# B3zaleel/draco-sharp

Measured on AMD Instinct MI355X. Metric: decoded_meshes_per_sec, higher is better.
Workload: dtype int32

## Files before the change

### draco-sharp_amd/csrc/dsa_kernels.h

```cpp
#pragma once
#include <hip/hip_runtime.h>
#include <stdint.h>

#include "dsa_common.h"
#include "dsa_locate.h"
#include "dsa_needs.h"
#ifdef DSA_EXPERIMENTS
#include "dsa_lanes.h"
#else
#define LN_FLAG_SYMBOLS 1u
#define LN_FLAG_PREDICT 2u
#define LN_FLAG_OCT 8u
namespace dsa { namespace lanes {
__device__ __forceinline__ bool ln_sym_eligible(const AttrDesc &, const MeshLayout &, uint32_t, uint32_t) { return false; }
__device__ __forceinline__ bool ln_oct_eligible(const AttrDesc &, uint32_t) { return false; }
} }
#endif

#ifndef DSA_CHAIN_PRIO
#define DSA_CHAIN_PRIO 3
#endif

namespace dsa {

__device__ __forceinline__ uint32_t cnext(uint32_t c) { return (c % 3u == 2u) ? c - 2u : c + 1u; }
__device__ __forceinline__ uint32_t cprev(uint32_t c) { return (c % 3u == 0u) ? c + 2u : c - 1u; }
__device__ __forceinline__ uint32_t uni(uint32_t v) { return (uint32_t)__builtin_amdgcn_readfirstlane((int)v); }
__device__ __forceinline__ uint32_t lane_id() { return threadIdx.x & 63u; }
template <class T>
__device__ __forceinline__ T *uni_ptr(T *p) {
  const uint64_t v = (uint64_t)p;
  return (T *)(((uint64_t)(uint32_t)__builtin_amdgcn_readfirstlane((int)(uint32_t)(v >> 32)) << 32) | (uint32_t)__builtin_amdgcn_readfirstlane((int)(uint32_t)v));
}
__device__ __forceinline__ uint32_t rdlane(uint32_t v, uint32_t l) { return (uint32_t)__builtin_amdgcn_readlane((int)v, (int)l); }
#define LATE_HANDOFF 0x40000u
__device__ __forceinline__ void late_handoff(uint8_t *arena, const MeshLayout &L, MeshDesc *D, uint32_t ai, uint32_t flags, uint32_t bit);
__device__ __forceinline__ uint64_t clk() { return __builtin_amdgcn_s_memtime(); }
__device__ __forceinline__ uint64_t realclk() { return __builtin_amdgcn_s_memrealtime(); }
__device__ __forceinline__ uint32_t leading_lanes(bool pred) { uint64_t m = ~__ballot(pred); return m ? (uint32_t)__builtin_ctzll(m) : 64u; }
#define WAIT_VM0() __builtin_amdgcn_s_waitcnt(0x0F70)

template <int CTRL>
__device__ __forceinline__ uint32_t dpp_mov(uint32_t x) { return (uint32_t)__builtin_amdgcn_update_dpp(0, (int)x, CTRL, 0xF, 0xF, false); }
__device__ __forceinline__ uint32_t lane_prev(uint32_t x) { return dpp_mov<0x138>(x); }
template <class Op>
__device__ __forceinline__ uint32_t wave_incl_scan(uint32_t x, Op op) {
  const uint32_t lane = lane_id(), rl = lane & 15u;
  uint32_t t;
  t = dpp_mov<0x111>(x); if (rl >= 1) x = op(t, x);
  t = dpp_mov<0x112>(x); if (rl >= 2) x = op(t, x);
  t = dpp_mov<0x114>(x); if (rl >= 4) x = op(t, x);
  t = dpp_mov<0x118>(x); if (rl >= 8) x = op(t, x);
  t = dpp_mov<0x142>(x); if ((lane & 31u) >= 16) x = op(t, x);
  t = dpp_mov<0x143>(x); if (lane >= 32) x = op(t, x);
  return x;
}
__device__ __forceinline__ uint32_t wave_excl_scan(uint32_t v, uint32_t *total) {
  const uint32_t x = wave_incl_scan(v, [](uint32_t a, uint32_t b) { return a + b; });
  *total = rdlane(x, 63);
  return x - v;
}

template <bool CP> struct Rec;
struct FaceIds { uint32_t v0, v1, v2, o0, o1, o2; };
template <> struct Rec<false> {
  static constexpr uint32_t WORDS = 8;
  struct Raw { uint4 v, o; };
  static __device__ __forceinline__ Raw load(const uint32_t *frec, uint32_t f) { Raw r; r.v = ((const uint4 *)frec)[(size_t)f * 2]; r.o = ((const uint4 *)frec)[(size_t)f * 2 + 1]; return r; }
  static __device__ __forceinline__ Raw none() { Raw r; r.v = make_uint4(0, 0, 0, 0); r.o = make_uint4(DSA_INVALID, DSA_INVALID, DSA_INVALID, 0); return r; }
  static __device__ __forceinline__ Raw or_none(bool ok, const Raw &x) { return ok ? x : none(); }
  static __device__ __forceinline__ uint32_t sel3(uint32_t k, uint32_t x, uint32_t y, uint32_t z) { return k == 0 ? x : (k == 1 ? y : z); }
  static __device__ __forceinline__ uint32_t vertex(const Raw &r, uint32_t k) { return sel3(k, r.v.x, r.v.y, r.v.z); }
  static __device__ __forceinline__ uint32_t opp(const Raw &r, uint32_t k) { return sel3(k, r.o.x, r.o.y, r.o.z); }
  static __device__ __forceinline__ uint32_t get_v(const uint32_t *frec, uint32_t c) { return frec[fv_idx(c)]; }
  static __device__ __forceinline__ uint32_t get_o(const uint32_t *frec, uint32_t c) { return frec[fo_idx(c)]; }
  static __device__ __forceinline__ uint32_t get_o_plain(const uint32_t *frec, uint32_t c) { return frec[fo_idx(c)]; }
  static __device__ __forceinline__ void set_v(uint32_t *frec, uint32_t c, uint32_t val) { frec[fv_idx(c)] = val; }
  static __device__ __forceinline__ void link(uint32_t *frec, uint32_t c, uint32_t val) { frec[fo_idx(c)] = val; }
  static __device__ __forceinline__ void link_lds(uint32_t *stage, uint32_t c_rel, uint32_t val) { stage[fo_idx(c_rel)] = val; }
  static __device__ __forceinline__ void store(uint32_t *frec, uint32_t f, const FaceIds &x) {
    ((uint4 *)frec)[(size_t)f * 2] = make_uint4(x.v0, x.v1, x.v2, 0u); ((uint4 *)frec)[(size_t)f * 2 + 1] = make_uint4(x.o0, x.o1, x.o2, 0u);
  }
  static __device__ __forceinline__ void store_lds(uint32_t *stage, uint32_t slot, const FaceIds &x) {
    *(uint4 *)&stage[slot * 8] = make_uint4(x.v0, x.v1, x.v2, 0u); *(uint4 *)&stage[slot * 8 + 4] = make_uint4(x.o0, x.o1, x.o2, 0u);
  }
  static __device__ __forceinline__ uint4 vertices_of(const uint32_t *frec, uint32_t f) { return ((const uint4 *)frec)[(size_t)f * 2]; }
};
template <> struct Rec<true> {
  static constexpr uint32_t WORDS = 4;
  static constexpr uint32_t M = 0x1FFFFFu;
  struct Raw { uint64_t v, o; };
  static __device__ __forceinline__ uint64_t pack(uint32_t a, uint32_t b, uint32_t c) { return (uint64_t)(a & M) | ((uint64_t)(b & M) << 21) | ((uint64_t)(c & M) << 42); }
  static __device__ __forceinline__ uint32_t field(uint64_t w, uint32_t k) { return (uint32_t)((int32_t)((uint32_t)(w >> (21u * k)) << 11) >> 11); }
  static __device__ __forceinline__ Raw load(const uint32_t *frec, uint32_t f) { const uint4 q = ((const uint4 *)frec)[f]; Raw r; r.v = (uint64_t)q.x | ((uint64_t)q.y << 32); r.o = (uint64_t)q.z | ((uint64_t)q.w << 32); return r; }
  static __device__ __forceinline__ Raw none() { Raw r; r.v = 0; r.o = ~0ull; return r; }
  static __device__ __forceinline__ Raw or_none(bool ok, const Raw &x) { Raw r; r.v = ok ? x.v : 0ull; r.o = ok ? x.o : ~0ull; return r; }
  static __device__ __forceinline__ uint32_t vertex(const Raw &r, uint32_t k) { return field(r.v, k); }
  static __device__ __forceinline__ uint32_t opp(const Raw &r, uint32_t k) { return field(r.o, k); }
  static __device__ __forceinline__ uint32_t get_v(const uint32_t *frec, uint32_t c) { return field(((const uint64_t *)frec)[(size_t)(c >> 2) * 2], c & 3u); }
  static __device__ __forceinline__ uint32_t get_o(const uint32_t *frec, uint32_t c) {
    return field(__hip_atomic_load((const unsigned long long *)frec + (size_t)(c >> 2) * 2 + 1, __ATOMIC_RELAXED, __HIP_MEMORY_SCOPE_AGENT), c & 3u);
  }
  static __device__ __forceinline__ uint32_t get_o_plain(const uint32_t *frec, uint32_t c) { return field(((const uint64_t *)frec)[(size_t)(c >> 2) * 2 + 1], c & 3u); }
  static __device__ __forceinline__ void set_v(uint32_t *frec, uint32_t c, uint32_t val) {
    uint64_t *w = (uint64_t *)frec + (size_t)(c >> 2) * 2;
    const uint32_t sh = 21u * (c & 3u);
    *w = (*w & ~((uint64_t)M << sh)) | ((uint64_t)(val & M) << sh);
  }
  static __device__ __forceinline__ void link(uint32_t *frec, uint32_t c, uint32_t val) {
    const uint32_t sh = 21u * (c & 3u);
    atomicAnd((unsigned long long *)frec + (size_t)(c >> 2) * 2 + 1, ((unsigned long long)(val & M) << sh) | ~((unsigned long long)M << sh));
  }
  static __device__ __forceinline__ void link_lds(uint32_t *stage, uint32_t c_rel, uint32_t val) {
    const uint32_t sh = 21u * (c_rel & 3u);
    atomicAnd((unsigned long long *)stage + (size_t)(c_rel >> 2) * 2 + 1, ((unsigned long long)(val & M) << sh) | ~((unsigned long long)M << sh));
  }
  static __device__ __forceinline__ uint4 quad(const FaceIds &x) { const uint64_t v = pack(x.v0, x.v1, x.v2), o = pack(x.o0, x.o1, x.o2); return make_uint4((uint32_t)v, (uint32_t)(v >> 32), (uint32_t)o, (uint32_t)(o >> 32)); }
  static __device__ __forceinline__ void store(uint32_t *frec, uint32_t f, const FaceIds &x) { ((uint4 *)frec)[f] = quad(x); }
  static __device__ __forceinline__ void store_lds(uint32_t *stage, uint32_t slot, const FaceIds &x) { *(uint4 *)&stage[slot * 4] = quad(x); }
  static __device__ __forceinline__ uint4 vertices_of(const uint32_t *frec, uint32_t f) {
    const uint64_t v = ((const uint64_t *)frec)[(size_t)f * 2];
    return make_uint4(field(v, 0), field(v, 1), field(v, 2), 0u);
  }
};
__device__ __forceinline__ uint32_t k_next(uint32_t k) { return k == 2u ? 0u : k + 1u; }
__device__ __forceinline__ uint32_t k_prev(uint32_t k) { return k == 0u ? 2u : k - 1u; }

__device__ __forceinline__ uint8_t *seam_block(uint8_t *arena, const MeshLayout &L, const SeamLayout &g, uint32_t d) {
  return arena + L.seam + g.data + (uint64_t)d * g.data_stride;
}
__device__ __forceinline__ const uint32_t *att_para(uint8_t *arena, const MeshLayout &L, const MeshDesc *D, const AttrDesc &a) {
  if (a.corner_data == 0) return (const uint32_t *)(arena + L.para);
  const SeamLayout g = seam_layout(L.cap_faces, L.cap_vertices, D->num_att_data, L.rec_compact != 0);
  return (const uint32_t *)(seam_block(arena, L, g, (uint32_t)a.corner_data - 1u) + g.para);
}


template <bool TOGGLE>
__device__ __forceinline__ uint32_t rabs_block_to_words(const Rabs &rb, uint32_t count, uint32_t *words) {
  uint32_t state = rb.state, left = rb.off, first = DSA_INVALID;
  const uint32_t p = rb.p;
  const uintptr_t a0 = (uintptr_t)rb.buf + (left ? left - 1u : 0u);
  const uint32_t *wp = (const uint32_t *)(a0 & ~(uintptr_t)3);
  uint32_t sh = (uint32_t)(a0 & 3u) * 8u;
  uint32_t cur = wp[0], nxt = wp[-1];
  uint32_t word = 0, last = 1;
  for (uint32_t i = 0; i < count; ++i) {
    if (state < 4096u && left > 0u) {
      state = state * 256u + ((cur >> sh) & 255u);
      --left;
      if (sh == 0u) { sh = 24u; cur = nxt; --wp; nxt = wp[-1]; } else sh -= 8u;
    }
    const uint32_t quot = state >> 8, rem = state & 255u, xn = quot * p;
    const bool val = rem < p;
    state = val ? xn + rem : state - xn - p;
    if (val && first == DSA_INVALID) first = i;
    if (TOGGLE) { last ^= val ? 0u : 1u; word |= last << (i & 31u); }
    else word |= (val ? 1u : 0u) << (i & 31u);
    if ((i & 31u) == 31u) { words[i >> 5] = word; word = 0; }
  }
  if (count & 31u) words[count >> 5] = word;
  return first;
}

__global__ __launch_bounds__(WAVE, 4) void k_locate(uint8_t *arena, const MeshLayout *layouts, MeshDesc *descs, uint32_t n, BatchGlobals *G) {
  uint32_t mesh = blockIdx.x;
  if (mesh >= n || threadIdx.x != 0) return;
  MeshDesc *D = &descs[mesh];
  locate_mesh(arena, layouts[mesh], D);
  if (D->status != ST_OK || D->general) return;
  locate_attribute_headers(arena, layouts[mesh], D);
  if (D->status != ST_OK) return;
  locate_attribute_values(arena, layouts[mesh], D, G, nullptr, nullptr, LOC_UNTIL_TAGS);
}
__global__ __launch_bounds__(WAVE, 4) void k_locate_resume(uint8_t *arena, const MeshLayout *layouts, MeshDesc *descs, uint32_t n, BatchGlobals *G) {
  __shared__ uint32_t s_cum[LOC_MAX_TAGS + 1];
  __shared__ __attribute__((aligned(16))) uint32_t s_lut[LOC_LDS_WORDS];
  uint32_t mesh = blockIdx.x;
  if (mesh >= n || threadIdx.x != 0) return;
  MeshDesc *D = &descs[mesh];
  if (D->status != ST_OK || D->general || !D->values_pending) return;
  if (D->values_pending == 2 && !D->seam_tables_done) return;
  locate_attribute_values(arena, layouts[mesh], D, G, s_cum, s_lut, LOC_RESUME);
}

#define CN_REC_BLOCKS 8
#define CN_STAGE 32
#define CN_WIN 64

#define CN_CTX_WORDS (6 * 64)
#define CN_LDS_WORDS (CN_STAGE * 8 + CN_REC_BLOCKS * 64 * 2 + CN_WIN + CN_CTX_WORDS)
#define VAL_LM(x_) ((x_) == DSA_INVALID ? DSA_INVALID : ((x_) & 0x1FFFFFu))
#define VAL_OF(x_) ((x_) >> 21)
__device__ __forceinline__ uint32_t val_pack(uint32_t lm, uint32_t val) { return (lm & 0x1FFFFFu) | ((val < 2047u ? val : 2047u) << 21); }
__device__ __forceinline__ bool valence_decode_list(MeshDesc *D, const uint8_t *stream, uint32_t stream_len, uint32_t off_table, uint32_t nsym, uint32_t P,
                                                    uint32_t off_rans, uint32_t size_rans, uint32_t count, uint32_t *out, uint32_t *sh_tmp) {
  const uint32_t lane = lane_id();
  const uint32_t precision = 1u << P, l_base = precision * 4;
  __syncthreads();
  if (lane == 0) { Rd r(stream, stream_len, off_table); if (!read_prob_table(r, nsym, sh_tmp)) fail(D, ST_INVALID, 400); }
  __syncthreads();
  if (status_of(D) != ST_OK) return false;
  const uint32_t pr = lane < nsym ? sh_tmp[lane] : 0u;
  uint32_t tot;
  const uint32_t ex = wave_excl_scan(pr, &tot);
  if (tot != precision) { if (lane == 0) fail(D, ST_INVALID, 401); return false; }
  const uint32_t cum = lane < nsym ? ex : precision;
// ... 1351 lines not shown
          if (pr) { if (k >= nsym) ok = false; else { lds_cum[k] = pr; symtab[k] = i; ++k; } }
        }
      }
      if (!ok || !r.ok || k != nsym) fail(D, ST_INVALID, 400);
    } else if (!read_prob_table(r, nsym, lds_cum)) fail(D, ST_INVALID, 400);
  }
  WAIT_VM0();
  __syncthreads();
  if (status_of(D) != ST_OK) return;
  uint32_t carry = 0;
  for (uint32_t b0 = 0; b0 < nsym; b0 += WAVE) {
    uint32_t i = b0 + lane;
    uint32_t pr = i < nsym ? lds_cum[i] : 0u;
    uint32_t tot;
    uint32_t ex = wave_excl_scan(pr, &tot);
    if (i < nsym) lds_cum[i] = carry + ex;
    carry += tot;
  }
  if (carry != precision) { if (lane == 0) fail(D, ST_INVALID, 401); return; }
  const uint32_t nblocks = (nsym + WAVE - 1) / WAVE;
  for (uint32_t i = nsym + lane; i < nblocks * WAVE + 1; i += WAVE) lds_cum[i] = precision;
  __syncthreads();
  uint32_t coarse = (lane < nblocks) ? lds_cum[lane * WAVE] : precision;
  uint32_t fine0 = lds_cum[lane];
  const uint8_t *buf = stream + a.off_rans;
  uint32_t x, off;
  {
    uint32_t st = 0, o = 0;
    bool ok = rans_init(buf, a.size_rans, l_base, &st, &o);
    if (!ok) { if (lane == 0) fail(D, ST_INVALID, 402); return; }
    x = uni(st); off = uni(o);
  }
  const uintptr_t base_addr = (uintptr_t)buf;
  const uint32_t mis = (uint32_t)(base_addr & 3u);
  const uint32_t *abuf = (const uint32_t *)(base_addr - mis);
  uint32_t chunk = 0xFFFFFFFFu, W = 0;
  const uint32_t mask = precision - 1;
  uint32_t mine = 0;
  for (uint32_t i = 0; i < num_values; ++i) {
    while (x < l_base && off > 0) {
      --off;
      uint32_t q = off + mis;
      uint32_t ch = q >> 8;
      if (ch != chunk) { chunk = ch; W = abuf[(size_t)ch * 64 + lane]; }
      uint32_t byte = (rdlane(W, (q & 255u) >> 2) >> ((q & 3u) * 8)) & 0xFFu;
      x = (x << 8) | byte;
    }
    uint32_t rem = x & mask;
    uint32_t s, cs, nx;
    if (nblocks == 1) {
      uint32_t j = (uint32_t)__popcll(__ballot(fine0 <= rem)) - 1u;
      cs = rdlane(fine0, j);
      nx = (j < 63) ? rdlane(fine0, j + 1) : precision;
      s = j;
    } else {
      uint32_t b = (uint32_t)__popcll(__ballot(coarse <= rem)) - 1u;
      uint32_t v = lds_cum[b * WAVE + lane];
      uint32_t j = (uint32_t)__popcll(__ballot(v <= rem)) - 1u;
      cs = rdlane(v, j);
      nx = (j < 63) ? rdlane(v, j + 1) : rdlane(coarse, b + 1);
      s = b * WAVE + j;
    }
    x = (nx - cs) * (x >> P) + rem - cs;
    if ((i & 63u) == lane) mine = s;
    if ((i & 63u) == 63u) out[i - 63u + lane] = mine;
  }
  uint32_t tail = num_values & 63u;
  if (tail && lane < tail) out[num_values - tail + lane] = mine;
  if (symtab) {
    WAIT_VM0();
    __syncthreads();
    for (uint32_t i = lane; i < num_values; i += WAVE) out[i] = symtab[out[i]];
  }
}

__device__ __forceinline__ void rans_decode_serial(MeshDesc *D, const uint8_t *stream, uint32_t stream_len, const AttrDesc &a, uint32_t num_values,
                                   uint32_t *out, uint32_t *cum ) {
  if (threadIdx.x != 0) return;
  const uint32_t nsym = a.num_symbols, P = a.precision_bits, precision = 1u << P, l_base = precision * 4;
  Rd r(stream, stream_len, a.off_table);
  if (!read_prob_table(r, nsym, cum)) { fail(D, ST_INVALID, 410); return; }
  uint32_t c = 0;
  for (uint32_t i = 0; i < nsym; ++i) { uint32_t pr = cum[i]; cum[i] = c; c += pr; if (c > precision) break; }
  if (c != precision) { fail(D, ST_INVALID, 411); return; }
  cum[nsym] = precision;
  const uint8_t *buf = stream + a.off_rans;
  uint32_t x, off;
  if (!rans_init(buf, a.size_rans, l_base, &x, &off)) { fail(D, ST_INVALID, 412); return; }
  for (uint32_t i = 0; i < num_values; ++i) {
    while (x < l_base && off > 0) x = (x << 8) | buf[--off];
    uint32_t rem = x & (precision - 1);
    uint32_t lo = 0, hi = nsym;
    while (hi - lo > 1) { uint32_t mid = (lo + hi) >> 1; if (cum[mid] <= rem) lo = mid; else hi = mid; }
    uint32_t cs = cum[lo];
    x = (cum[lo + 1] - cs) * (x >> P) + rem - cs;
    out[i] = lo;
  }
}

typedef uint32_t v32u __attribute__((ext_vector_type(32)));

#define SYM_EARLY_FUSE 0x400u
__device__ __forceinline__ void predict_wave(uint8_t *arena, const MeshLayout &L, MeshDesc *D, uint32_t ai, uint32_t phase, uint32_t flags);
__device__ __forceinline__ void predict_wrap_attribute(uint8_t *arena, const MeshLayout &L, MeshDesc *D, uint32_t ai, uint32_t phase, uint32_t flags);
__device__ __forceinline__ void finalize_attribute(uint8_t *arena, const MeshLayout &L, const MeshDesc *D, uint32_t ai, uint32_t phase, uint32_t flags, uint32_t tid, uint32_t stride);
__device__ __forceinline__ void early_tail(uint8_t *arena, const MeshLayout &L, MeshDesc *D, uint32_t ai, uint32_t flags) {
  if (!(flags & SYM_EARLY_FUSE) || D->general) return;
  const AttrDesc &a = D->att[ai];
  if (att_is_late(a)) return;
  WAIT_VM0();
  __threadfence_block();
  __syncthreads();
  if (status_of(D) != ST_OK) return;
  predict_wrap_attribute(arena, L, D, ai, 0u, flags);
  predict_wave(arena, L, D, ai, 0u, flags);
  WAIT_VM0();
  __threadfence_block();
  __syncthreads();
  if (status_of(D) != ST_OK) return;
  finalize_attribute(arena, L, D, ai, 0u, flags, lane_id(), WAVE);
  if (lane_id() == 0) D->att[ai].early_done = 1;
}

__device__ __forceinline__ void late_handoff(uint8_t *arena, const MeshLayout &L, MeshDesc *D, uint32_t ai, uint32_t flags, uint32_t bit) {
  if (!(flags & LATE_HANDOFF) || D->general) return;
  AttrDesc &a = D->att[ai];
  if (!wrap_fast_ok(a, flags) || !att_is_late(a) || att_behind_tables(a) || a.pred_kind != 1) return;
  __builtin_amdgcn_fence(__ATOMIC_RELEASE, "agent");
  __syncthreads();
  uint32_t old = 0;
  if (lane_id() == 0) old = __hip_atomic_fetch_or(&a.late_ready, bit, __ATOMIC_ACQ_REL, __HIP_MEMORY_SCOPE_AGENT);
  old = uni(old);
  if (!(old & (3u ^ bit))) return;
  __builtin_amdgcn_fence(__ATOMIC_ACQUIRE, "agent");
  if (status_of(D) != ST_OK) return;
  predict_wrap_attribute(arena, L, D, ai, 1u, flags);
  WAIT_VM0();
  __syncthreads();
  if (lane_id() == 0) a.late_ready = 7u;
}

#define REG_ATTR 0
#define REG_TAGS 1
#define REG_VLIST 2
#define REG_SCRATCH_BYTES (4096u * 6u + REG_MAX_SYMS * 4u)
#ifdef DSA_SYM_STAMPS
#define REG_STAMP_BEGIN() uint64_t st_t = clk()
#define REG_STAMP(p) { const uint64_t t_ = clk(); if (ATTR && ai < 3 && lane_id() == 0) { const uint32_t k_ = 3u * (p) + ai; \
    ((uint16_t *)D->dbg)[k_ < 6 ? 20 + k_ : 30 + k_] = (uint16_t)((t_ - st_t) >> 10 > 65535 ? 65535 : (t_ - st_t) >> 10); } st_t = t_; }
#else
#define REG_STAMP_BEGIN()
#define REG_STAMP(p)
#endif
__device__ __forceinline__ uint32_t reg_final_symbol(uint32_t v, bool positive) {
  return positive ? v : ((v & 1u) ? (uint32_t)(-(int32_t)(v >> 1) - 1) : (v >> 1));
}
template <int MODE>
__device__ __forceinline__ void reg_decode_stream(uint8_t *arena, const MeshLayout &L, MeshDesc *D, uint32_t ai, uint32_t flags) {
  constexpr bool TAGS = MODE == REG_TAGS, VLIST = MODE == REG_VLIST, ATTR = MODE == REG_ATTR;
  AttrDesc &a = D->att[VLIST ? 0u : ai];
  uint8_t *scratch;
  REG_STAMP_BEGIN();
  uint32_t st_off_table = a.off_table, st_off_rans = a.off_rans, st_size_rans = a.size_rans, st_nsym = a.num_symbols;
  uint32_t st_values = a.num_entries * (TAGS ? 1u : (uint32_t)a.nc_portable);
  uint32_t *out = (uint32_t *)(arena + L.work[VLIST ? 0u : ai]);
  if (VLIST) {
    st_values = D->val_count[ai];
    if (st_values == 0 || D->val_prec[ai] != 12 || D->val_nsym[ai] > 64) return;
    if ((uint64_t)L.rec_compact * 16ull * D->num_faces < 6ull * REG_SCRATCH_BYTES) return;
    st_off_table = D->val_off_table[ai]; st_off_rans = D->val_off_rans[ai]; st_size_rans = D->val_size_rans[ai]; st_nsym = D->val_nsym[ai];
    uint32_t before = 0;
    for (uint32_t k = 0; k < ai; ++k) before += D->val_count[k];
    if ((uint64_t)before + st_values > 3ull * D->num_faces) return;
    out = (uint32_t *)(arena + L.faces) + before;
    scratch = arena + L.frec + (size_t)ai * REG_SCRATCH_BYTES;
  } else if (TAGS) {
    if (a.source != SRC_TAGGED || a.tags_done || a.num_symbols > LOC_MAX_TAGS || a.num_distinct <= 1 || a.num_entries == 0) return;
    const uint64_t slots = ((uint64_t)a.num_entries * 4 + 15) & ~15ull;
    if ((uint64_t)L.work_cap[ai] * 4 < slots + REG_SCRATCH_BYTES) return;
    scratch = arena + L.work[ai] + slots;
  } else {
    if (lanes::ln_sym_eligible(a, L, ai, flags)) return;
    if (sym_filtered(a, flags)) return;
    if (!sym_reg_eligible(a, L, ai)) return;
    scratch = arena + L.out[ai];
  }
  const uint8_t *stream = arena + L.stream;
  uint32_t *slot_tab = (uint32_t *)scratch;
  uint16_t *slot_sym = (uint16_t *)(scratch + 4096 * 4);
  uint32_t *lds = (uint32_t *)(scratch + 4096 * 6);
  const uint32_t lane = lane_id();
  const uint32_t nsym = uni(st_nsym);
  const uint32_t num_values = uni(st_values);
  if (num_values == 0) return;
  if (lane == 0) {
    Rd r(stream, L.stream_len, st_off_table);
    if (!read_prob_table(r, nsym, lds)) fail(D, ST_INVALID, 400);
  }
  __syncthreads();
  if (status_of(D) != ST_OK) return;
  uint32_t carry = 0, one_at = DSA_INVALID;
  bool over = false;
  for (uint32_t b0 = 0; b0 < REG_MAX_SYMS; b0 += WAVE) {
    uint32_t i = b0 + lane;
    uint32_t pr = i < nsym ? lds[i] : 0u;
    if (pr > 4095) { over = true; one_at = i; }
    uint32_t tot;
    uint32_t ex = wave_excl_scan(pr, &tot);
    lds[i] = (pr << 12) | ((carry + ex) & 4095u);
    carry += tot;
    if (carry > 4096) over = true;
  }
  if (VLIST && carry == 4096 && __ballot(over)) {
    uint32_t st = 0, o = 0;
    if (!rans_init(stream + st_off_rans, st_size_rans, 16384, &st, &o)) { if (lane == 0) fail(D, ST_INVALID, 402); return; }
    const uint32_t one = (uint32_t)__builtin_ctzll(__ballot(one_at != DSA_INVALID));
    const uint32_t sym = rdlane(one_at, one);
    for (uint32_t i = lane; i < num_values; i += WAVE) out[i] = sym;
    WAIT_VM0();
    __syncthreads();
    if (lane == 0) atomicOr(&D->val_lists_done, 1u << ai);
    return;
  }
  if (__ballot(over) || carry != 4096) { if (lane == 0) fail(D, carry != 4096 ? ST_INVALID : ST_NOTIMPL, 401); return; }
  __syncthreads();
  for (uint32_t sy = lane; sy < nsym; sy += WAVE) {
    const uint32_t e = lds[sy], f = e >> 12, c = e & 4095u;
    for (uint32_t j = 0; j < f; ++j) { slot_tab[c + j] = f | (j << 16); slot_sym[c + j] = (uint16_t)sy; }
  }
  WAIT_VM0();
  __syncthreads();
  v32u tab_lo, tab_hi;
#pragma unroll
  for (int k = 0; k < 32; ++k) { tab_lo[k] = slot_tab[k * WAVE + lane]; tab_hi[k] = slot_tab[(k + 32) * WAVE + lane]; }
  const uint8_t *buf = stream + st_off_rans;
  uint32_t x, off;
  {
    uint32_t st = 0, o = 0;
    bool ok = rans_init(buf, st_size_rans, 16384, &st, &o);
    if (!ok) { if (lane == 0) fail(D, ST_INVALID, 402); return; }
    x = uni(st); off = uni(o);
  }
  const uint32_t mis = (uint32_t)((L.stream + st_off_rans) & 3u);
  const uint32_t *abuf = (const uint32_t *)(arena + (L.stream + st_off_rans - mis));
  uint32_t chunk = 0x7FFFFFFFu, W = 0;
  uint32_t next_chunk = 0x7FFFFFFFu, Wn = 0;
  uint32_t mine = 0;
  uint32_t pend = 0;
  const bool positive = ATTR && a.have_scheme && (a.pred_transform == 2 || a.pred_transform == 3);
  WAIT_VM0();
  REG_STAMP(0);
  uint64_t P = (uint64_t)x << 32;
  uint32_t rc = 0;
  uint32_t dl = 0;
  bool exhausted = false;
  for (uint32_t i0 = 0; i0 < num_values; i0 += WAVE) {
    const uint32_t cnt = uni(num_values - i0 < WAVE ? num_values - i0 : WAVE);
    uint32_t j = 0;
    while (j < cnt) {
      if (!exhausted) {
        {
          uint32_t k6, va, vf;
          uint32_t js = uni(j);
          asm volatile(
              " s_getpc_b64 s[22:23]\n"
              "Lupc%=:\n"
              " s_mul_i32 %[k6], %[j], Lus1_%=-Lus0_%=\n"
              " s_add_u32 s22, s22, Lus0_%=-Lupc%=\n"
              " s_addc_u32 s23, s23, 0\n"
              " s_add_u32 s22, s22, %[k6]\n"
              " s_addc_u32 s23, s23, 0\n"
              " s_set_gpr_idx_on s22, gpr_idx(SRC1)\n"
              " s_setpc_b64 s[22:23]\n"
              ".irp J,0,1,2,3,4,5,6,7,8,9,10,11,12,13,14,15,16,17,18,19,20,21,22,23,24,25,26,27,28,29,30,31,32,33,34,35,36,37,38,39,40,41,42,43,44,45,46,47,48,49,50,51,52,53,54,55,56,57,58,59,60,61,62,63\n"
              "Lus\\J\\()_%=:\n"
              " s_cmpk_lt_u32 s21, 0x4000\n"
              " s_cbranch_scc1 Lur\\J\\()_%=\n"
              "Lok\\J\\()_%=:\n"
              " s_bfe_u32 %[k6], s21, 0x60006\n"
              " s_set_gpr_idx_idx %[k6]\n"
              " v_lshrrev_b32_e64 %[vf], 12, s21\n"
              " v_mul_u32_u24_sdwa %[va], %[vf], v16 dst_sel:DWORD dst_unused:UNUSED_PAD src0_sel:DWORD src1_sel:WORD_0\n"
              " v_add_u32_sdwa %[va], %[va], v16 dst_sel:DWORD dst_unused:UNUSED_PAD src0_sel:DWORD src1_sel:WORD_1\n"
              " v_writelane_b32 %[mine], s21, \\J\n"
              " v_readlane_b32 s21, %[va], s21\n"
              ".endr\n"
              " s_movk_i32 %[j], 64\n"
              " s_branch Luend%=\n"
              ".irp J,0,1,2,3,4,5,6,7,8,9,10,11,12,13,14,15,16,17,18,19,20,21,22,23,24,25,26,27,28,29,30,31,32,33,34,35,36,37,38,39,40,41,42,43,44,45,46,47,48,49,50,51,52,53,54,55,56,57,58,59,60,61,62,63\n"
              "Lur\\J\\()_%=:\n"
              " s_sub_u32 %[rc], %[rc], 1\n"
              " s_cbranch_scc1 Lue\\J\\()_%=\n"
              " s_lshl_b64 s[20:21], s[20:21], 8\n"
              " s_cmpk_lt_u32 s21, 0x4000\n"
              " s_cbranch_scc0 Lok\\J\\()_%=\n"
              " s_branch Lur\\J\\()_%=\n"
              "Lue\\J\\()_%=:\n"
              " s_cmp_lt_u32 %[off], 4\n"
              " s_cbranch_scc1 Lsl\\J\\()_%=\n"
              " s_sub_u32 %[dl], %[dl], 1\n"
              " s_cbranch_scc1 Lsl\\J\\()_%=\n"
              " v_readlane_b32 s20, %[W], %[dl]\n"
              " s_sub_u32 %[off], %[off], 4\n"
              " s_mov_b32 %[rc], 3\n"
              " s_lshl_b64 s[20:21], s[20:21], 8\n"
              " s_cmpk_lt_u32 s21, 0x4000\n"
              " s_cbranch_scc0 Lok\\J\\()_%=\n"
              " s_branch Lur\\J\\()_%=\n"
              "Lsl\\J\\()_%=:\n"
              " s_movk_i32 %[j], \\J\n"
              " s_branch Luempty%=\n"
              ".endr\n"
              "Luempty%=:\n"
              " s_mov_b32 %[rc], 0\n"
              "Luend%=:\n"
              " s_set_gpr_idx_off\n"
              : "+{s[20:21]}"(P), [rc] "+s"(rc), [j] "+s"(js), [mine] "+v"(mine), [k6] "=&s"(k6), [va] "=&v"(va), [vf] "=&v"(vf),
                [off] "+s"(off), [dl] "+s"(dl)
              : "{v[16:47]}"(tab_lo), "{v[48:79]}"(tab_hi), [W] "v"(W)
              : "vcc", "scc", "s22", "s23");
          j = js;
        }
        if (j < cnt) {
          if (off == 0) exhausted = true;
          else {
            const uint32_t end = off + mis;
            const uint32_t d = (end - 1) >> 2, r = end - 4 * d, ch = d >> 6;
            if (ch != chunk) {
              if (next_chunk == ch) W = Wn;
              else { W = abuf[(size_t)ch * 64 + lane]; WAIT_VM0(); }
              chunk = ch;
            }
            const uint32_t res = rdlane(W, d & 63u) << (8 * (4 - r));
            rc = uni(r < off ? r : off);
            off -= rc;
            dl = uni(d & 63u);
            P = (P & 0xFFFFFFFF00000000ull) | res;
          }
        }
      } else {
        const uint32_t xs = uni((uint32_t)(P >> 32));
        mine = (lane == j) ? xs : mine;
        const uint32_t k5 = (xs >> 6) & 31u, l6 = xs & 63u;
        const uint32_t e0 = rdlane(tab_lo[k5], l6), e1 = rdlane(tab_hi[k5], l6);
        const uint32_t e = (xs & 2048u) ? e1 : e0;
        P = (uint64_t)((e & 0xFFFFu) * (xs >> 12) + (e >> 16)) << 32;
        ++j;
      }
    }
    if (ATTR) { if (i0) out[i0 - WAVE + lane] = reg_final_symbol(pend, positive); }
    else if (lane < cnt) out[i0 + lane] = mine;
    if (chunk != 0x7FFFFFFFu && chunk != 0 && next_chunk != chunk - 1) { next_chunk = chunk - 1; Wn = abuf[next_chunk * 64u + lane]; }
    if (ATTR) pend = slot_sym[mine & 4095u];
  }
  REG_STAMP(1);
  if (ATTR) {
    const uint32_t last = (num_values - 1) & ~(WAVE - 1u);
    if (lane < num_values - last) out[last + lane] = reg_final_symbol(pend, positive);
  }
  WAIT_VM0();
  __syncthreads();
  if (VLIST) {
    for (uint32_t i = lane; i < num_values; i += WAVE) out[i] = slot_sym[out[i] & 4095u];
    WAIT_VM0();
    __syncthreads();
    if (lane == 0) atomicOr(&D->val_lists_done, 1u << ai);
    return;
  }
  if (TAGS) {
    uint8_t *tags = arena + L.out[ai];
    uint64_t bits = 0;
    uint32_t worst = 0;
    const uint32_t nc = a.nc_portable;
    for (uint32_t i = lane; i < num_values; i += WAVE) {
      const uint32_t v = slot_sym[out[i] & 4095u];
      tags[i] = (uint8_t)v;
      bits += (uint64_t)v * nc;
      worst = v > worst ? v : worst;
    }
    for (int d = 32; d >= 1; d >>= 1) {
      bits += ((uint64_t)(uint32_t)__shfl_xor((int)(uint32_t)(bits >> 32), d, WAVE) << 32) | (uint32_t)__shfl_xor((int)(uint32_t)bits, d, WAVE);
      const uint32_t w2 = (uint32_t)__shfl_xor((int)worst, d, WAVE);
      worst = w2 > worst ? w2 : worst;
    }
    WAIT_VM0();
    __syncthreads();
    if (lane == 0) { a.table = (bits & 0x00FFFFFFFFFFFFFFull) | ((uint64_t)(worst > 255u ? 255u : worst) << 56); a.tags_done = 1; }
    return;
  }
  REG_STAMP(2);
  early_tail(arena, L, D, ai, flags);
  late_handoff(arena, L, D, ai, flags, 1u);
}

__global__ __launch_bounds__(WAVE, 6) void k_symbols_reg(uint8_t *arena, const MeshLayout *layouts, MeshDesc *descs, uint32_t n, uint32_t flags) {
  uint32_t mesh = blockIdx.x, ai = blockIdx.y;
  if (mesh >= n) return;
  MeshDesc *D = &descs[mesh];
  if (D->status != ST_OK || D->general || ai >= D->num_attributes) return;
  reg_decode_stream<REG_ATTR>(arena, layouts[mesh], D, ai, flags);
}
__global__ __launch_bounds__(WAVE, 6) void k_tags(uint8_t *arena, const MeshLayout *layouts, MeshDesc *descs, uint32_t n) {
  uint32_t mesh = blockIdx.x;
  if (mesh >= n) return;
  MeshDesc *D = &descs[mesh];
  if (D->status != ST_OK || D->general || !D->values_pending || D->resume_att >= D->num_attributes) return;
  if (D->values_pending == 2) return;
  reg_decode_stream<REG_TAGS>(arena, layouts[mesh], D, D->resume_att, 0u);
}
__global__ __launch_bounds__(WAVE, 6) void k_valence_lists(uint8_t *arena, const MeshLayout *layouts, MeshDesc *descs, uint32_t n) {
  uint32_t mesh = blockIdx.x, c = blockIdx.y;
  if (mesh >= n) return;
  MeshDesc *D = &descs[mesh];
  if (D->status != ST_OK || D->general || D->encoder_type == 0 || D->traversal_type != 2) return;
  reg_decode_stream<REG_VLIST>(arena, layouts[mesh], D, c, 0u);
}


__global__ __launch_bounds__(WAVE) void k_symbols_wide(uint8_t *arena, const MeshLayout *layouts, MeshDesc *descs, uint32_t n, uint32_t flags) {
  const uint32_t mesh = blockIdx.x, ai = blockIdx.y;
  if (mesh >= n) return;
  MeshDesc *D = &descs[mesh];
  if (D->status != ST_OK || D->general || ai >= D->num_attributes) return;
  const MeshLayout &L = layouts[mesh];
  const AttrDesc &a = D->att[ai];
  if (a.source == SRC_BYTES) return;
  if (lanes::ln_sym_eligible(a, L, ai, flags)) return;
  if (sym_filtered(a, flags)) return;
  if (!sym_wide_eligible(a, L, ai)) return;
  const uint32_t lane = lane_id();
  const uint32_t num_values = a.num_entries * a.nc_portable;
  if (num_values == 0) return;
  const uint8_t *stream = arena + L.stream;
  const uint32_t stream_len = L.stream_len;
  uint32_t *out = (uint32_t *)(arena + L.work[ai]);
  const bool compact = a.num_symbols > SYM_MAX_LDS;
  const uint32_t nsym = compact ? a.num_distinct : a.num_symbols;
  uint32_t *symtab = compact ? (uint32_t *)(arena + a.table) : nullptr;
  uint32_t *gtab = compact ? symtab + nsym : (uint32_t *)(arena + L.out[ai]);
  const uint32_t P = a.precision_bits, precision = 1u << P, l_base = precision * 4;
  if (lane == 0) {
    Rd r(stream, stream_len, a.off_table);
    uint32_t k = 0;
    bool ok = true;
    for (uint32_t i = 0; i < a.num_symbols && ok; ++i) {
      const uint32_t pd = r.u8(), token = pd & 3u;
      if (token == 3u) {
        const uint32_t offset = pd >> 2;
        if (i + offset >= a.num_symbols) ok = false;
        if (!compact) for (uint32_t j = 0; j <= offset && i + j < a.num_symbols; ++j) gtab[i + j] = 0;
        i += offset;
      } else {
        uint32_t pr = pd >> 2;
        for (uint32_t j = 0; j < token; ++j) pr |= r.u8() << (8 * (j + 1) - 2);
        if (compact) { if (pr) { if (k >= nsym) ok = false; else { gtab[k] = pr; symtab[k] = i; ++k; } } }
        else gtab[i] = pr;
      }
    }
    if (!ok || !r.ok || (compact && k != nsym)) fail(D, ST_INVALID, 400);
    WAIT_VM0();
    __threadfence_block();
  }
  __syncthreads();
  if (status_of(D) != ST_OK) return;
  uint32_t carry = 0;
  for (uint32_t b0 = 0; b0 < nsym; b0 += WAVE) {
    const uint32_t i = b0 + lane;
    const uint32_t pr = i < nsym ? gtab[i] : 0u;
    uint32_t tot;
    const uint32_t ex = wave_excl_scan(pr, &tot);
    if (i < nsym) gtab[i] = carry + ex;
    carry += tot;
  }
  if (carry != precision) { if (lane == 0) fail(D, ST_INVALID, 401); return; }
  if (lane == 0) gtab[nsym] = precision;
  WAIT_VM0();
  __threadfence_block();
  __syncthreads();
  const uint32_t nblocks = (nsym + WAVE - 1) / WAVE;
  const bool hand = uni(P) <= 15u;
  v32u tab;
#pragma unroll
  for (int r = 0; r < 32; ++r) {
    const uint32_t i = (uint32_t)r * WAVE + lane;
    const uint32_t c0 = i < nsym ? gtab[i] : 0x1FFFFu, c1 = i < nsym ? gtab[i + 1] : 0x1FFFFu;
    tab[r] = (i < nsym && c0 < 0x10000u && !(hand && c0 >= precision)) ? (hand ? ((c0 << 16) | (c1 - c0)) : (c0 | ((c1 - c0) << 16))) : 0xFFFFFFFFu;
  }
  const uint32_t coarse = lane < nblocks ? gtab[lane * WAVE] : 0xFFFFFFFFu;
  const uint8_t *buf = stream + a.off_rans;
  uint32_t x, off;
  {
    uint32_t st = 0, o = 0;
    const bool ok = rans_init(buf, a.size_rans, l_base, &st, &o);
    if (!ok) { if (lane == 0) fail(D, ST_INVALID, 402); return; }
    x = uni(st); off = uni(o);
  }
  const uintptr_t base_addr = (uintptr_t)buf;
  const uint32_t mis = (uint32_t)(base_addr & 3u);
  const uint32_t *abuf = (const uint32_t *)(base_addr - mis);
  uint32_t chunk = 0xFFFFFFFFu, W = 0;
  const uint32_t mask = precision - 1;
  uint32_t mine = 0;
  if (hand) {
    uint64_t PR = (uint64_t)x << 32;
    uint32_t rc = 0, dl = 0;
    bool exhausted = false;
    const uint32_t lb = uni(l_base), mk = uni(mask), pb = uni(P);
    uint32_t best = 0;
#pragma unroll
    for (int r = 0; r < 32; ++r) {
      const uint32_t w = tab[r], k = w == 0xFFFFFFFFu ? 0u : (((w & 0xFFFFu) << 11) | (uint32_t)(31 - r) << 6 | (63u - lane));
      best = k > best ? k : best;
    }
    for (int d = 32; d >= 1; d >>= 1) { const uint32_t o = (uint32_t)__shfl_xor((int)best, d, WAVE); best = o > best ? o : best; }
    const uint32_t idom = uni((31u - ((best >> 6) & 31u)) * WAVE + (63u - (best & 63u)));
    const uint32_t fdom = uni(best >> 11), cdom = uni(gtab[idom]), tdom = uni(idom + WAVE);
    WAIT_VM0();
    for (uint32_t i0 = 0; i0 < num_values; i0 += WAVE) {
      const uint32_t cnt = uni(num_values - i0 < WAVE ? num_values - i0 : WAVE);
      uint32_t j = 0;
      while (j < cnt) {
        if (!exhausted) {
          {
            uint32_t k6, rem, key, bb, q, t, jj, e, f, tmp;
            uint32_t js = uni(j);
            rc = uni(rc); off = uni(off); dl = uni(dl);
            PR = ((uint64_t)uni((uint32_t)(PR >> 32)) << 32) | uni((uint32_t)PR);
            asm volatile(
                " s_getpc_b64 s[22:23]\n"
                "Lwpc%=:\n"
                " s_mul_i32 %[k6], %[j], Lws1_%=-Lws0_%=\n"
                " s_add_u32 s22, s22, Lws0_%=-Lwpc%=\n"
                " s_addc_u32 s23, s23, 0\n"
                " s_add_u32 s22, s22, %[k6]\n"
                " s_addc_u32 s23, s23, 0\n"
                " s_set_gpr_idx_on s22, gpr_idx(SRC1)\n"
                " s_setpc_b64 s[22:23]\n"
                ".irp J,0,1,2,3,4,5,6,7,8,9,10,11,12,13,14,15,16,17,18,19,20,21,22,23,24,25,26,27,28,29,30,31,32,33,34,35,36,37,38,39,40,41,42,43,44,45,46,47,48,49,50,51,52,53,54,55,56,57,58,59,60,61,62,63\n"
                "Lws\\J\\()_%=:\n"
                " s_cmp_lt_u32 s21, %[lb]\n"
                " s_cbranch_scc1 Lwr\\J\\()_%=\n"
                "Lwk\\J\\()_%=:\n"
                " s_and_b32 %[rem], s21, %[mk]\n"
                " s_sub_u32 %[e], %[rem], %[cdom]\n"
                " s_cmp_lt_u32 %[e], %[fdom]\n"
                " s_cbranch_scc0 Lwq\\J\\()_%=\n"
                " s_lshr_b32 %[q], s21, %[pb]\n"
                " s_mul_i32 %[q], %[q], %[fdom]\n"
                " v_writelane_b32 %[mine], %[tdom], \\J\n"
                " s_add_u32 s21, %[q], %[e]\n"
                "Lwn\\J\\()_%=:\n"
                ".endr\n"
                " s_movk_i32 %[j], 64\n"
                " s_branch Lwend%=\n"
                ".irp J,0,1,2,3,4,5,6,7,8,9,10,11,12,13,14,15,16,17,18,19,20,21,22,23,24,25,26,27,28,29,30,31,32,33,34,35,36,37,38,39,40,41,42,43,44,45,46,47,48,49,50,51,52,53,54,55,56,57,58,59,60,61,62,63\n"
                "Lwq\\J\\()_%=:\n"
                " v_cmp_le_u32_e64 vcc, %[coarse], %[rem]\n"
                " s_pack_ll_b32_b16 %[key], 0xffff, %[rem]\n"
                " s_lshr_b32 %[q], s21, %[pb]\n"
                " s_bcnt1_i32_b64 %[bb], vcc\n"
                " s_set_gpr_idx_idx %[bb]\n"
// ... 896 lines not shown
```

Measured before the change: 111,400.

## Build rANS slot table via wave max-scan instead of per-symbol serial fill

New measurement: 111,300. No clear change (-0.1%).

```diff
diff --git a/draco-sharp_amd/csrc/dsa_kernels.h b/draco-sharp_amd/csrc/dsa_kernels.h
--- a/draco-sharp_amd/csrc/dsa_kernels.h
+++ b/draco-sharp_amd/csrc/dsa_kernels.h
@@ -32,6 +32,12 @@
   const uint64_t v = (uint64_t)p;
   return (T *)(((uint64_t)(uint32_t)__builtin_amdgcn_readfirstlane((int)(uint32_t)(v >> 32)) << 32) | (uint32_t)__builtin_amdgcn_readfirstlane((int)(uint32_t)v));
 }
+template <class T>
+__device__ __forceinline__ __attribute__((address_space(1))) T *uni_global(T *p) {
+  const uint64_t v = (uint64_t)p;
+  return (__attribute__((address_space(1))) T *)(((uint64_t)(uint32_t)__builtin_amdgcn_readfirstlane((int)(uint32_t)(v >> 32)) << 32) |
+                                                 (uint32_t)__builtin_amdgcn_readfirstlane((int)(uint32_t)v));
+}
 __device__ __forceinline__ uint32_t rdlane(uint32_t v, uint32_t l) { return (uint32_t)__builtin_amdgcn_readlane((int)v, (int)l); }
 #define LATE_HANDOFF 0x40000u
 __device__ __forceinline__ void late_handoff(uint8_t *arena, const MeshLayout &L, MeshDesc *D, uint32_t ai, uint32_t flags, uint32_t bit);
@@ -53,6 +59,16 @@
   t = dpp_mov<0x118>(x); if (rl >= 8) x = op(t, x);
   t = dpp_mov<0x142>(x); if ((lane & 31u) >= 16) x = op(t, x);
   t = dpp_mov<0x143>(x); if (lane >= 32) x = op(t, x);
+  return x;
+}
+__device__ __forceinline__ uint32_t wave_incl_max(uint32_t x) {
+  uint32_t t;
+  t = dpp_mov<0x111>(x); x = t > x ? t : x;
+  t = dpp_mov<0x112>(x); x = t > x ? t : x;
+  t = dpp_mov<0x114>(x); x = t > x ? t : x;
+  t = dpp_mov<0x118>(x); x = t > x ? t : x;
+  t = dpp_mov<0x142>(x); x = t > x ? t : x;
+  t = dpp_mov<0x143>(x); x = t > x ? t : x;
   return x;
 }
 __device__ __forceinline__ uint32_t wave_excl_scan(uint32_t v, uint32_t *total) {
@@ -1710,6 +1726,19 @@
 #define REG_STAMP_BEGIN()
 #define REG_STAMP(p)
 #endif
+#if defined(DSA_SYM_SETUP_STAMPS) && defined(DSA_SYM_STAMPS)
+#error "DSA_SYM_STAMPS and DSA_SYM_SETUP_STAMPS share the dbg half-words: one per build"
+#endif
+#ifdef DSA_SYM_SETUP_STAMPS
+#define REG_SUB_BEGIN() uint64_t sub_t = clk(); uint64_t sub_w = 0
+#define REG_SUB(s) { const uint64_t t_ = clk(), d_ = (t_ - sub_t) >> 10; sub_w |= (d_ > 4095 ? 4095ull : d_) << (12 * (s)); sub_t = t_; }
+#define REG_SUB_END() { if (ATTR && ai < 3 && lane_id() == 0) { uint16_t *h_ = (uint16_t *)D->dbg + (ai < 2 ? 20 + 3 * ai : 36); \
+    h_[0] = (uint16_t)sub_w; h_[1] = (uint16_t)(sub_w >> 16); h_[2] = (uint16_t)(sub_w >> 32); } }
+#else
+#define REG_SUB_BEGIN()
+#define REG_SUB(s)
+#define REG_SUB_END()
+#endif
 __device__ __forceinline__ uint32_t reg_final_symbol(uint32_t v, bool positive) {
   return positive ? v : ((v & 1u) ? (uint32_t)(-(int32_t)(v >> 1) - 1) : (v >> 1));
 }
@@ -1730,7 +1759,7 @@
     uint32_t before = 0;
     for (uint32_t k = 0; k < ai; ++k) before += D->val_count[k];
     if ((uint64_t)before + st_values > 3ull * D->num_faces) return;
-    out = (uint32_t *)(arena + L.faces) + before;
+    out = (uint32_t *)(arena + L.faces) + uni(before);
     scratch = arena + L.frec + (size_t)ai * REG_SCRATCH_BYTES;
   } else if (TAGS) {
     if (a.source != SRC_TAGGED || a.tags_done || a.num_symbols > LOC_MAX_TAGS || a.num_distinct <= 1 || a.num_entries == 0) return;
@@ -1751,15 +1780,18 @@
   const uint32_t nsym = uni(st_nsym);
   const uint32_t num_values = uni(st_values);
   if (num_values == 0) return;
+  REG_SUB_BEGIN();
+  for (uint32_t k = 0; k < 4096; k += WAVE) slot_tab[k + lane] = 0u;
   if (lane == 0) {
     Rd r(stream, L.stream_len, st_off_table);
     if (!read_prob_table(r, nsym, lds)) fail(D, ST_INVALID, 400);
   }
   __syncthreads();
   if (status_of(D) != ST_OK) return;
+  REG_SUB(0);
   uint32_t carry = 0, one_at = DSA_INVALID;
   bool over = false;
-  for (uint32_t b0 = 0; b0 < REG_MAX_SYMS; b0 += WAVE) {
+  for (uint32_t b0 = 0; b0 < nsym; b0 += WAVE) {
     uint32_t i = b0 + lane;
     uint32_t pr = i < nsym ? lds[i] : 0u;
     if (pr > 4095) { over = true; one_at = i; }
@@ -1782,15 +1814,61 @@
   }
   if (__ballot(over) || carry != 4096) { if (lane == 0) fail(D, carry != 4096 ? ST_INVALID : ST_NOTIMPL, 401); return; }
   __syncthreads();
+  REG_SUB(1);
+  WAIT_VM0();
   for (uint32_t sy = lane; sy < nsym; sy += WAVE) {
-    const uint32_t e = lds[sy], f = e >> 12, c = e & 4095u;
-    for (uint32_t j = 0; j < f; ++j) { slot_tab[c + j] = f | (j << 16); slot_sym[c + j] = (uint16_t)sy; }
+    const uint32_t e = lds[sy];
+    if (e >> 12) slot_tab[e & 4095u] = sy + 1u;
   }
   WAIT_VM0();
   __syncthreads();
   v32u tab_lo, tab_hi;
-#pragma unroll
-  for (int k = 0; k < 32; ++k) { tab_lo[k] = slot_tab[k * WAVE + lane]; tab_hi[k] = slot_tab[(k + 32) * WAVE + lane]; }
+  {
+    uint32_t t[64];
+    const __attribute__((address_space(1))) uint32_t *marks[4];
+    __attribute__((address_space(1))) uint16_t *syms[2];
+#pragma unroll
+    for (int q = 0; q < 4; ++q) marks[q] = uni_global(slot_tab + q * 1024);
+#pragma unroll
+    for (int q = 0; q < 2; ++q) syms[q] = uni_global(slot_sym + q * 2048);
+#pragma unroll
+    for (int k = 0; k < 64; ++k) t[k] = (marks[k >> 4] + lane)[(k & 15) * WAVE];
+    uint32_t before = 0;
+#pragma unroll
+    for (int k = 0; k < 64; ++k) {
+      uint32_t m = wave_incl_max(t[k]);
+      m = m > before ? m : before;
+      before = rdlane(m, 63);
+      const uint32_t sy = (m - 1u) & 4095u;
+      (syms[k >> 5] + lane)[(k & 31) * WAVE] = (uint16_t)sy;
+      t[k] = lds[sy];
+      __builtin_amdgcn_sched_barrier(0);
+    }
+#pragma unroll
+    for (int k = 0; k < 64; ++k) {
+      t[k] = (t[k] >> 12) | ((lane - (t[k] & 4095u) + (uint32_t)k * WAVE) << 16);
+      if ((k & 7) == 7) __builtin_amdgcn_sched_barrier(0);
+    }
+#pragma unroll
+    for (int k = 0; k < 32; ++k) { tab_lo[k] = t[k]; tab_hi[k] = t[k + 32]; }
+  }
+#ifdef DSA_SYM_TABLE_CHECK
+  {
+    WAIT_VM0();
+    __syncthreads();
+    bool differs = false;
+    for (uint32_t sy = lane; sy < nsym; sy += WAVE) {
+      const uint32_t e = lds[sy], f = e >> 12, c = e & 4095u;
+      for (uint32_t j = 0; j < f; ++j) { slot_tab[c + j] = f | (j << 16); if (slot_sym[c + j] != (uint16_t)sy) differs = true; }
+    }
+    WAIT_VM0();
+    __syncthreads();
+#pragma unroll
+    for (int k = 0; k < 32; ++k) if (tab_lo[k] != slot_tab[k * WAVE + lane] || tab_hi[k] != slot_tab[(k + 32) * WAVE + lane]) differs = true;
+    if (__ballot(differs)) { if (lane == 0) fail(D, ST_INVALID, 409); return; }
+  }
+#endif
+  REG_SUB(2);
   const uint8_t *buf = stream + st_off_rans;
   uint32_t x, off;
   {
@@ -1807,6 +1885,8 @@
   uint32_t pend = 0;
   const bool positive = ATTR && a.have_scheme && (a.pred_transform == 2 || a.pred_transform == 3);
   WAIT_VM0();
+  REG_SUB(3);
+  REG_SUB_END();
   REG_STAMP(0);
   uint64_t P = (uint64_t)x << 32;
   uint32_t rc = 0;
@@ -1919,7 +1999,9 @@
   WAIT_VM0();
   __syncthreads();
   if (VLIST) {
-    for (uint32_t i = lane; i < num_values; i += WAVE) out[i] = slot_sym[out[i] & 4095u];
+    uint32_t first = lane;
+    asm volatile("" : "+v"(first));
+    for (uint32_t i = first; i < num_values; i += WAVE) out[i] = slot_sym[out[i] & 4095u];
     WAIT_VM0();
     __syncthreads();
     if (lane == 0) atomicOr(&D->val_lists_done, 1u << ai);
@@ -1964,7 +2046,7 @@
   MeshDesc *D = &descs[mesh];
   if (D->status != ST_OK || D->general || !D->values_pending || D->resume_att >= D->num_attributes) return;
   if (D->values_pending == 2) return;
-  reg_decode_stream<REG_TAGS>(arena, layouts[mesh], D, D->resume_att, 0u);
+  reg_decode_stream<REG_TAGS>(arena, layouts[mesh], D, uni(D->resume_att), 0u);
 }
 __global__ __launch_bounds__(WAVE, 6) void k_valence_lists(uint8_t *arena, const MeshLayout *layouts, MeshDesc *descs, uint32_t n) {
   uint32_t mesh = blockIdx.x, c = blockIdx.y;
```
